# nii-yamagishilab/NELE-GAN

Measured on AMD Instinct MI355X. Metric: utterances/sec per GAN_epoch step (G+D+metric loss), higher is better.
Workload: dtype bf16

## Files before the change

nele_gan_amd/_lib.py:

```python
import ctypes
import os

import torch

from . import _abi, _abi_ext, _abi_ext2, _abi_ext3

FUNCS = dict(_abi.FUNCS, **_abi_ext.FUNCS)
CONSTS = dict(_abi.CONSTS, **_abi_ext.CONSTS)
FUNCS2 = dict(_abi_ext2.FUNCS)
CONSTS2 = dict(_abi_ext2.CONSTS)
FUNCS3 = dict(_abi_ext3.FUNCS)
CONSTS3 = dict(_abi_ext3.CONSTS)

_HERE = os.path.dirname(os.path.abspath(__file__))
LIB_PATH = os.environ.get('NELE_LIB') or os.path.join(_HERE, 'libnele_hip.so')

c_int = ctypes.c_int
c_float = ctypes.c_float
c_double = ctypes.c_double
c_void_p = ctypes.c_void_p
c_size_t = ctypes.c_size_t
c_longlong = ctypes.c_longlong


class NeleError(RuntimeError):
    pass


def _load():
    if not os.path.exists(LIB_PATH):
        raise ImportError(
            "nele_gan_amd: %s not found -- build it with `python -c 'import __graft_entry__ as g; g.build()'` "
            "or `make -C nele_gan_amd/csrc` (hipcc, gfx950). There is no fallback path." % LIB_PATH)
    return ctypes.CDLL(LIB_PATH)


lib = _load()


def _bind(every):
    missing = sorted(n for n in every if not hasattr(lib, n))
    if missing:
        raise ImportError("nele_gan_amd: %s does not export %s (declared in include/nele_hip*.h) -- "
                          "rebuild it with `python -c 'import __graft_entry__ as g; g.build()'`" % (LIB_PATH, ', '.join(missing)))
    sigs = {}
    for name, (restype, argtypes) in every.items():
        fn = getattr(lib, name)
        fn.restype = getattr(ctypes, 'c_' + restype)
        fn.argtypes = sigs[name] = [getattr(ctypes, 'c_' + a) for a in argtypes]
    return sigs


_SIGS = _bind(dict(FUNCS, **FUNCS2))
_SIGS3 = _bind(FUNCS3)


def check(status, name=''):
    if status != 0:
        msg = lib.nele_last_error_string().decode('utf-8', 'replace')
        if status == -1:
            raise ValueError("%s: %s" % (name, msg))
        raise NeleError("%s failed (status %d): %s" % (name, status, msg))


PLAN_MAXARGS = CONSTS['NELE_PLAN_MAXARGS']


class nele_plan_job(ctypes.Structure):
    _fields_ = [('op', c_int), ('nargs', c_int), ('stream', c_int), ('slot', c_int * PLAN_MAXARGS), ('ival', c_longlong * PLAN_MAXARGS),
                ('fval', c_double * PLAN_MAXARGS)]


def call(name, *args):
    check(getattr(lib, name)(*args), name)


def ptr(t):
    if t is None:
        return None
    if not t.is_cuda:
        raise ValueError("nele_gan_amd: expected a tensor on the GPU (got %s)" % t.device)
    if not t.is_contiguous():
        raise ValueError("nele_gan_amd: expected a contiguous tensor")
    return c_void_p(t.data_ptr())


def norm_dev(dev):
    dev = torch.device(dev)
    if dev.type == 'cuda' and dev.index is None:
        dev = torch.device('cuda', torch.cuda.current_device())
    return dev


_raw_stream = getattr(torch._C, '_cuda_getCurrentRawStream', None)
_raw_device = getattr(torch._C, '_cuda_getDevice', None)


def stream():
    if _raw_stream is not None and _raw_device is not None:
        return c_void_p(_raw_stream(_raw_device()))
    return c_void_p(torch.cuda.current_stream().cuda_stream)


def profile_begin(tag):
    lib.nele_profile_begin(tag.encode() if tag else None)


# ... 19 lines not shown
```

nele_gan_amd/csrc/conv16.hip:

```cpp
#include "conv_common.h"
#include <cstdlib>
#include <cstring>
#include <type_traits>

#define C16_TW 64
#ifndef C16_SB
#define C16_SB 4
#endif

#ifdef C16_PROF
__device__ unsigned long long c16_prof[8];
#define C16_T(var) const unsigned long long var = __builtin_readcyclecounter()
#define C16_ACC(slot, t0_, t1_) do { c16_acc[slot] += (t1_) - (t0_); } while (0)
#else
#define C16_T(var) do {} while (0)
#define C16_ACC(slot, t0_, t1_) do {} while (0)
#endif

struct Conv16Args {
    const __bf16* A;
    const __bf16* Wfrag;
    const float* bias;
    const __bf16* aux;
    void* out;
    int N, epi;
    float slope;
    int KH, KW, sps, nsteps;
    int RSP, NR;
    int lgC, swz_sh, swz_mask;
    int ntiles, TH;
    double* gap;
    const int* wvalid;
    ConvGeom g;
};

__device__ __forceinline__ void c16_dma(const __bf16* gsrc_lane, __bf16* lds_piece) {
    __builtin_amdgcn_global_load_lds((const __attribute__((address_space(1))) void*)gsrc_lane, (__attribute__((address_space(3))) void*)lds_piece, 16, 0, 0);
}

template <int TN, int TH, bool OUT16>
__global__ __launch_bounds__(256, 2) void conv16_kernel(Conv16Args p) {
    C16_T(t_start);
#ifdef C16_PROF
    unsigned long long c16_acc[5] = {0, 0, 0, 0, 0};
#endif
    extern __shared__ __attribute__((aligned(16))) __bf16 lds16[];
    const ConvGeom& g = p.g;
    const int tid = threadIdx.x, lane = tid & 63, li = lane & 15, lg = lane >> 4;
    const int wave = __builtin_amdgcn_readfirstlane(tid >> 6);
    int wo0, ho0, b;
    {
        const int ntw = (g.Wout + C16_TW - 1) / C16_TW, nth = (g.Hout + TH - 1) / TH;
        const int per = (int)((gridDim.x + 7) >> 3);
        const int tile = (int)(blockIdx.x & 7) * per + (int)(blockIdx.x >> 3);
        if (tile >= p.ntiles) return;
        const int tw_i = tile % ntw, rem = tile / ntw;
        wo0 = tw_i * C16_TW; ho0 = (rem % nth) * TH; b = rem / nth;
    }
    const int C = g.C, RSP = p.RSP, NR = p.NR;
    const int wcols = C16_TW + p.KW - 1;
    const int nrows = TH + p.KH - 1;
    const int hi0 = ho0 + g.ih0, wi0 = wo0 + g.iw0;
    const int vcols = max(1, min(wcols, g.W - wi0));
    const int vrows = max(1, min(nrows, g.H - hi0));
    const __bf16* abase = p.A + (((size_t)b * g.H + hi0) * g.W + wi0) * C;
    __bf16* wring = lds16 + NR * RSP + 64;
    constexpr int CH = C16_SB * TN * 512;

    const int npieces = RSP >> 9;
    int rsrc[3];
#pragma unroll
    for (int t = 0; t < 3; ++t) {
        const int o = 512 * (wave + 4 * t) + 8 * lane;
        const int q = o / C, un = ((o - q * C) >> 3) ^ ((q >> p.swz_sh) & p.swz_mask);
        rsrc[t] = min(q, vcols - 1) * C + 8 * un;
    }
    auto row_dma = [&](int r) {
        const __bf16* src = abase + (size_t)min(r, vrows - 1) * g.W * C;
        __bf16* dst = lds16 + (r % NR) * RSP;
#pragma unroll
        for (int t = 0; t < 3; ++t)
            if (wave + 4 * t < npieces) c16_dma(src + rsrc[t], dst + 512 * (wave + 4 * t));
    };
    const int nchunk = (p.nsteps + C16_SB - 1) / C16_SB;
    const __bf16* wsrc = p.Wfrag + 512 * wave + 8 * lane;
    auto w_dma = [&](int c) {
        const __bf16* src = wsrc + (size_t)c * CH;
        __bf16* dst = wring + (c & 1) * CH + 512 * wave;
#pragma unroll
        for (int q = 0; q < (C16_SB * TN + 3) / 4; ++q)
            if ((C16_SB * TN) % 4 == 0 || wave + 4 * q < C16_SB * TN) c16_dma(src + 2048 * q, dst + 2048 * q);
    };
    int resident = min(NR, nrows) - 1;
    for (int r = 0; r <= resident; ++r) row_dma(r);
    w_dma(0);
    if (tid < 8) *reinterpret_cast<bf16x8*>(lds16 + NR * RSP + 8 * tid) = (bf16x8){(__bf16)0.f, (__bf16)0.f, (__bf16)0.f, (__bf16)0.f, (__bf16)0.f, (__bf16)0.f, (__bf16)0.f, (__bf16)0.f};

    const int nr = min(TH, g.Hout - ho0), ncol = min(4, (g.Wout - wo0 + 15) >> 4), total = nr * ncol;
    const int NPr = (total + 3) >> 2;
    const int n0 = 4 * TN * lg;
    const int vb = li * C;

    auto run = [&](auto np_tag) {
        constexpr int NP = decltype(np_tag)::value;
        int prow[NP], pcol[NP];
        bool pok[NP];
#pragma unroll
        for (int k = 0; k < NP; ++k) {
            int t = wave + 4 * k;
            pok[k] = t < total;
            if (!pok[k]) t -= total;
            if (t >= total) t %= total;
            prow[k] = t / ncol; pcol[k] = t - prow[k] * ncol;
        }
        f32x4 acc[NP][TN];
#pragma unroll
        for (int k = 0; k < NP; ++k)
#pragma unroll
            for (int j = 0; j < TN; ++j) acc[k][j] = (f32x4){0.f, 0.f, 0.f, 0.f};
        __builtin_amdgcn_s_waitcnt(0x0f70);
        __syncthreads();
        C16_T(t_pro);
        C16_ACC(1, t_start, t_pro);

        int lu = 0, rr[NP], so[NP];
#pragma unroll
        for (int k = 0; k < NP; ++k) { rr[k] = prow[k]; so[k] = prow[k] * RSP + 16 * pcol[k] * C; }
        const __bf16* wl = wring + lane * 8;
        auto ldfrag = [&](int uu, bf16x8 (&af)[NP], bf16x8 (&bfr)[TN]) {
            const int kk8 = lu * 32 + 8 * lg;
            const int vk = (vb + kk8) ^ ((((li + (kk8 >> p.lgC)) >> p.swz_sh) & p.swz_mask) << 3);
#pragma unroll
            for (int j = 0; j < TN; ++j) bfr[j] = *reinterpret_cast<const bf16x8*>(wl + (uu * TN + j) * 512);
#pragma unroll
            for (int k = 0; k < NP; ++k) af[k] = *reinterpret_cast<const bf16x8*>(lds16 + so[k] + vk);
            if (__builtin_expect(++lu == p.sps, 0)) {
                asm volatile("" ::: "memory");
                lu = 0;
#pragma unroll
                for (int k = 0; k < NP; ++k) {
                    so[k] += RSP;
                    if (++rr[k] == NR) { rr[k] = 0; so[k] -= NR * RSP; }
                }
            }
        };
        auto mm = [&](const bf16x8 (&af)[NP], const bf16x8 (&bfr)[TN]) {
#pragma unroll
            for (int k = 0; k < NP; ++k)
#pragma unroll
                for (int j = 0; j < TN; ++j) acc[k][j] = __builtin_amdgcn_mfma_f32_16x16x32_bf16(bfr[j], af[k], acc[k][j], 0, 0, 0);
        };
        constexpr int MPR = (NP * TN) / (NP + TN) > 0 ? (NP * TN) / (NP + TN) : 1;
#define C16_INTERLEAVE()                                                                  \
    _Pragma("unroll") for (int q_ = 0; q_ < NP + TN; ++q_) {                              \
        __builtin_amdgcn_sched_group_barrier(0x008, MPR, 0);                              \
        __builtin_amdgcn_sched_group_barrier(0x100, 1, 0);                                \
        __builtin_amdgcn_sched_group_barrier(0x002, 3, 0);                                \
    }                                                                                     \
    __builtin_amdgcn_sched_group_barrier(0x008, NP * TN, 0);                              \
    __builtin_amdgcn_sched_barrier(0);                                                    \
    __builtin_amdgcn_s_waitcnt(0xc07f);                                                   \
    __builtin_amdgcn_sched_barrier(0)
        const int nfull = p.nsteps / C16_SB, nrem = p.nsteps - nfull * C16_SB;
        int nl_row = (2 * C16_SB - 1) / p.sps, nl_rem = (2 * C16_SB - 1) - nl_row * p.sps;
        for (int c = 0; c < nfull; ++c) {
            if (c + 1 < nchunk) {
                w_dma(c + 1);
                const int need = min(nl_row + TH - 1, nrows - 1);
                if (need > resident) { ++resident; row_dma(resident); }
                nl_rem += C16_SB;
                while (nl_rem >= p.sps) { nl_rem -= p.sps; ++nl_row; }
            }
            bf16x8 a0[NP], b0[TN], a1[NP], b1[TN];
            ldfrag(0, a0, b0);
            __builtin_amdgcn_sched_barrier(0);
            __builtin_amdgcn_s_waitcnt(0xc07f);
            __builtin_amdgcn_sched_barrier(0);
#pragma unroll
            for (int uu = 0; uu + 1 < C16_SB; ++uu) {
                if (uu & 1) { ldfrag(uu + 1, a0, b0); mm(a1, b1); }
                else { ldfrag(uu + 1, a1, b1); mm(a0, b0); }
                C16_INTERLEAVE();
            }
            if (C16_SB & 1) mm(a0, b0); else mm(a1, b1);
            wl += (c & 1) ? -CH : CH;
            if (c + 1 < nchunk) {
                C16_T(t_w0);
                __builtin_amdgcn_s_waitcnt(0x0f70);
                C16_T(t_w1);
                __syncthreads();
                C16_T(t_w2);
                C16_ACC(2, t_w0, t_w1);
                C16_ACC(3, t_w1, t_w2);
            }
        }
#undef C16_INTERLEAVE
        for (int uu = 0; uu < nrem; ++uu) {
            bf16x8 a0[NP], b0[TN];
            ldfrag(uu, a0, b0);
            mm(a0, b0);
        }

        C16_T(t_epi);
        float bv[4 * TN];
#pragma unroll
        for (int q = 0; q < 4 * TN; ++q)
            bv[q] = ((p.epi == EPI_BIAS || p.epi == EPI_BIAS_LRELU) && n0 + q < p.N) ? p.bias[n0 + q] : 0.f;
        const bool pool = p.gap != nullptr;
        const int wpool = pool ? (p.wvalid ? min(p.wvalid[b], g.Wout) : g.Wout) : 0;
        double gs[4 * TN];
#pragma unroll
        for (int q = 0; q < 4 * TN; ++q) gs[q] = 0.0;
#pragma unroll
        for (int k = 0; k < NP; ++k) {
            const int ho = ho0 + prow[k], wo = wo0 + 16 * pcol[k] + li;
            if (!pok[k] || wo >= g.Wout || n0 >= p.N) continue;
            float v[4 * TN];
#pragma unroll
            for (int j = 0; j < TN; ++j)
#pragma unroll
                for (int reg = 0; reg < 4; ++reg) v[4 * j + reg] = acc[k][j][reg] + bv[4 * j + reg];
            if (p.epi == EPI_BIAS_LRELU) {
#pragma unroll
                for (int q = 0; q < 4 * TN; ++q) v[q] = v[q] > 0.f ? v[q] : p.slope * v[q];
                if (pool && wo < wpool) {
#pragma unroll
                    for (int q = 0; q < 4 * TN; ++q) gs[q] += (double)v[q];
                }
            } else if (p.epi == EPI_MASK_LRELU_GRAD) {
                const __bf16* xp = p.aux + (((size_t)b * g.Hout + ho) * g.Wout + wo) * p.N + n0;
#pragma unroll
                for (int j = 0; j < TN; ++j) {
                    if (n0 + 4 * j < p.N) {
                        const bf16x4 x = *reinterpret_cast<const bf16x4*>(xp + 4 * j);
#pragma unroll
                        for (int reg = 0; reg < 4; ++reg) v[4 * j + reg] = (float)x[reg] > 0.f ? v[4 * j + reg] : p.slope * v[4 * j + reg];
                    }
                }
            }
            const size_t o_off = (((size_t)b * g.OH + ho + g.oh0) * g.OW + wo + g.ow0) * g.OC + n0;
            if (OUT16) {
                __bf16* op = reinterpret_cast<__bf16*>(p.out) + o_off;
#pragma unroll
                for (int j = 0; j < TN; ++j) {
                    if (n0 + 4 * j < p.N) {
                        bf16x4 h;
#pragma unroll
                        for (int reg = 0; reg < 4; ++reg) h[reg] = (__bf16)v[4 * j + reg];
                        *reinterpret_cast<bf16x4*>(op + 4 * j) = h;
                    }
                }
            } else {
                float* op = reinterpret_cast<float*>(p.out) + o_off;
#pragma unroll
                for (int j = 0; j < TN; ++j)
                    if (n0 + 4 * j < p.N) *reinterpret_cast<float4*>(op + 4 * j) = make_float4(v[4 * j], v[4 * j + 1], v[4 * j + 2], v[4 * j + 3]);
            }
        }
        if (pool) {
            const int ntw_ = (g.Wout + C16_TW - 1) / C16_TW, nth_ = (g.Hout + TH - 1) / TH;
            const int part = ((ho0 / TH) * ntw_ + wo0 / C16_TW) * 4 + wave;
            double* gp = p.gap + ((size_t)b * (ntw_ * nth_ * 4) + part) * p.N + n0;
#pragma unroll
            for (int q = 0; q < 4 * TN; ++q) {
                const double t = row16_sum_dpp(gs[q]);
                if (li == 0 && n0 + q < p.N) gp[q] = t;
            }
        }
        C16_T(t_end);
        C16_ACC(4, t_epi, t_end);
        C16_ACC(0, t_start, t_end);
#ifdef C16_PROF
        if (threadIdx.x == 0) { for (int q_ = 0; q_ < 5; ++q_) atomicAdd(&c16_prof[q_], c16_acc[q_]); atomicAdd(&c16_prof[5], 1ull); }
#endif
    };
    if (TH == 8) {
        switch (NPr) {
            case 8: run(std::integral_constant<int, (TH == 8 ? 8 : 1)>{}); break;
            case 7: run(std::integral_constant<int, (TH == 8 ? 7 : 1)>{}); break;
            case 6: run(std::integral_constant<int, (TH == 8 ? 6 : 1)>{}); break;
            case 5: run(std::integral_constant<int, (TH == 8 ? 5 : 1)>{}); break;
            case 4: run(std::integral_constant<int, 4>{}); break;
            case 3: run(std::integral_constant<int, 3>{}); break;
            case 2: run(std::integral_constant<int, 2>{}); break;
            default: run(std::integral_constant<int, 1>{}); break;
        }
    } else {
        switch (NPr) {
            case 4: run(std::integral_constant<int, 4>{}); break;
            case 3: run(std::integral_constant<int, 3>{}); break;
            case 2: run(std::integral_constant<int, 2>{}); break;
            default: run(std::integral_constant<int, 1>{}); break;
        }
    }
}

__global__ __launch_bounds__(256) void conv16_pointwise_kernel(const float4* __restrict__ in, const float* __restrict__ W, const float* __restrict__ bias,
                                                               __bf16* __restrict__ out, long long M, float slope) {
    __shared__ float w[8][4], bs[8];
    if (threadIdx.x < 32) w[threadIdx.x >> 2][threadIdx.x & 3] = W[threadIdx.x];
    if (threadIdx.x < 8) bs[threadIdx.x] = bias[threadIdx.x];
    __syncthreads();
    for (long long m = (long long)blockIdx.x * 256 + threadIdx.x; m < M; m += (long long)gridDim.x * 256) {
        const float4 a = in[m];
        bf16x8 h;
#pragma unroll
        for (int n = 0; n < 8; ++n) {
            float v = fmaf(a.w, w[n][3], fmaf(a.y, w[n][1], fmaf(a.z, w[n][2], a.x * w[n][0]))) + bs[n];
            v = v > 0.f ? v : slope * v;
            h[n] = (__bf16)v;
        }
        *reinterpret_cast<bf16x8*>(out + 8 * m) = h;
    }
}

extern "C" int nele_conv16_pointwise_fwd(const float* in, const float* Wf, const float* bias, void* out16, long long M, int N, float slope, void* stream) {
    NELE_CHECK_ARG(in && Wf && bias && out16 && M > 0 && N == 8, "nele_conv16_pointwise_fwd: needs 4 -> 8 channels");
    const long long blocks = (M + 255) / 256;
    hipLaunchKernelGGL(conv16_pointwise_kernel, dim3((unsigned)(blocks < 8192 ? blocks : 8192)), dim3(256), 0, as_stream(stream),
                       reinterpret_cast<const float4*>(in), Wf, bias, reinterpret_cast<__bf16*>(out16), M, slope);
    NELE_CHECK_LAUNCH("conv16_pointwise_kernel");
    return NELE_OK;
}

struct C16FragJobs { const float* Wg[16]; __bf16* Wfrag[16]; int N[16], Ktot[16], seglen[16], KH[16]; };
__global__ void conv16_frag_kernel(C16FragJobs J) {
    const int job = blockIdx.y;
    const float* __restrict__ Wg = J.Wg[job];
    __bf16* __restrict__ Wf = J.Wfrag[job];
    const int N = J.N[job], Ktot = J.Ktot[job], seglen = J.seglen[job], KH = J.KH[job];
    const int TN = (N + 15) >> 4, sps = (seglen + 31) >> 5;
    const long long total = (long long)(KH * sps + C16_SB) * TN * 512;
    for (long long idx = (long long)blockIdx.x * blockDim.x + threadIdx.x; idx < total; idx += (long long)gridDim.x * blockDim.x) {
        const int e = (int)(idx & 7), lane = (int)((idx >> 3) & 63);
        const long long f = idx >> 9;
        const int j = (int)(f % TN), s = (int)(f / TN);
        const int m = lane & 15, gq = lane >> 4;
        const int n = 4 * TN * (m >> 2) + 4 * j + (m & 3);
        float v = 0.f;
        if (s < KH * sps && n < N) {
            const int kh = s / sps, us = s - kh * sps;
            const int ko = us * 32 + 8 * gq + e;
            if (ko < seglen) v = Wg[(size_t)n * Ktot + kh * seglen + ko];
        }
        Wf[idx] = (__bf16)v;
    }
}

struct C16Plan { int TN, TH, NR, RSP, lgC, swz_sh, swz_mask, sps; size_t lds; };
static bool c16_plan(int N, const ConvGeom& g, int KH, int KW, C16Plan* pl, int epi = EPI_NONE) {
    if (N < 4 || N > 64 || (N & 3) || g.C < 8 || g.C > 64 || (g.C & 7) || KH < 2 || KW < 2 || KW > 9 || KH > 9) return false;
    if (g.seglen != KW * g.C || g.Ktot != KH * KW * g.C) return false;
    C16Plan q;
    q.TN = (N + 15) >> 4;
    q.sps = (g.seglen + 31) >> 5;
    const int nsteps = KH * q.sps;
    int th = (nsteps * q.TN <= 64 && q.TN <= 2) ? 8 : 4;
    if (epi == EPI_MASK_LRELU_GRAD) th = 4;
    q.TH = th;
    q.lgC = 0; q.swz_sh = 0; q.swz_mask = 0;
    if (g.C == 64) { q.lgC = 6; q.swz_mask = 7; }
    else if (g.C == 32) { q.lgC = 5; q.swz_sh = 1; q.swz_mask = 3; }
    q.RSP = ((C16_TW + KW - 1) * g.C + 511) & ~511;
    if (q.RSP > 12 * 512) return false;
    const int full = q.TH + KH - 1;
    const int ring = q.sps >= 2 * C16_SB - 1 ? q.TH + 1 : q.sps >= C16_SB ? q.TH + 2 : full;
    q.NR = ring < full ? ring : full;
    q.lds = ((size_t)q.NR * q.RSP + 64 + 2 * C16_SB * q.TN * 512) * 2;
    if (q.lds > 160 * 1024) return false;
    *pl = q;
    return true;
}

#ifdef C16_PROF
extern "C" int nele_conv16_prof_read(unsigned long long* out8, int reset) {
    if (hipDeviceSynchronize() != hipSuccess) return 1;
    if (hipMemcpyFromSymbol(out8, HIP_SYMBOL(c16_prof), sizeof(unsigned long long) * 8) != hipSuccess) return 1;
    if (reset) { unsigned long long z[8] = {0}; if (hipMemcpyToSymbol(HIP_SYMBOL(c16_prof), z, sizeof(z)) != hipSuccess) return 1; }
    return 0;
}
#endif

extern "C" int nele_conv16_supported(int M, int N, const int* geom, int KH, int KW) {
    ConvGeom g;
    memcpy(&g, geom, sizeof(ConvGeom));
    C16Plan pl;
    return c16_plan(N, g, KH, KW, &pl) ? 1 : 0;
}

extern "C" long long nele_conv16_wfrag_elems(int N, int seglen, int KH) {
    const int TN = (N + 15) >> 4, sps = (seglen + 31) >> 5;
    return (long long)(KH * sps + C16_SB) * TN * 512;
}

extern "C" int nele_conv16_weight_prep_batch(const void* const* ptrs_host, const int* dims_host, int jobs, void* stream) {
    NELE_CHECK_ARG(ptrs_host && dims_host && jobs >= 1 && jobs <= 16, "nele_conv16_weight_prep_batch: 1..16 jobs");
    C16FragJobs J;
    long long mx = 0;
    for (int i = 0; i < jobs; ++i) {
        J.Wg[i] = (const float*)ptrs_host[2 * i]; J.Wfrag[i] = (__bf16*)ptrs_host[2 * i + 1];
        J.N[i] = dims_host[4 * i]; J.Ktot[i] = dims_host[4 * i + 1]; J.seglen[i] = dims_host[4 * i + 2]; J.KH[i] = dims_host[4 * i + 3];
        NELE_CHECK_ARG(J.Wg[i] && J.Wfrag[i] && J.Ktot[i] == J.seglen[i] * J.KH[i], "nele_conv16_weight_prep_batch: bad job %d", i);
        const long long t = nele_conv16_wfrag_elems(J.N[i], J.seglen[i], J.KH[i]);
        if (t > mx) mx = t;
    }
    const int blocks = (int)((mx + 255) / 256 < 512 ? (mx + 255) / 256 : 512);
    hipLaunchKernelGGL(conv16_frag_kernel, dim3(blocks, jobs), dim3(256), 0, as_stream(stream), J);
    NELE_CHECK_LAUNCH("conv16_frag_kernel");
    return NELE_OK;
}

template <int TN, int TH, bool OUT16>
static void c16_launch(const Conv16Args& a, dim3 grid, size_t lds, hipStream_t s) {
    static unsigned long long attr = 0;
    if (nele_first_use_on_device(&attr)) {
        (void)hipFuncSetAttribute(reinterpret_cast<const void*>(conv16_kernel<TN, TH, OUT16>), hipFuncAttributeMaxDynamicSharedMemorySize, 160 * 1024);
    }
    hipLaunchKernelGGL((conv16_kernel<TN, TH, OUT16>), grid, dim3(256), lds, s, a);
}

static int conv16_impl(const void* A16, const void* Wfrag, const float* bias, const void* aux16, void* out, int out_bf16, int M, int N, int epi,
                       float slope, const int* geom, int KH, int KW, const int* wvalid, double* gap_part, void* stream) {
    NELE_CHECK_ARG(A16 && Wfrag && out && geom, "nele_conv16: null pointer");
    ConvGeom g;
    memcpy(&g, geom, sizeof(ConvGeom));
    C16Plan pl;
    if (!c16_plan(N, g, KH, KW, &pl, epi)) return nele_set_error(NELE_ERR_UNSUPPORTED, "nele_conv16: unsupported geometry (C %d N %d %dx%d)", g.C, N, KH, KW);
    NELE_CHECK_ARG(epi == EPI_NONE || epi == EPI_BIAS || epi == EPI_BIAS_LRELU || epi == EPI_MASK_LRELU_GRAD, "nele_conv16: epilogue %d", epi);
    NELE_CHECK_ARG(epi != EPI_MASK_LRELU_GRAD || aux16, "nele_conv16: the mask epilogue needs the forward activation");
    NELE_CHECK_ARG((epi != EPI_BIAS && epi != EPI_BIAS_LRELU) || bias, "nele_conv16: bias missing");
    NELE_CHECK_ARG(g.Hout > 0 && g.Wout > 0 && M % (g.Hout * g.Wout) == 0, "nele_conv16: M is not a multiple of Hout * Wout");
    NELE_CHECK_ARG((g.OC & 3) == 0, "nele_conv16: output channel stride must be a multiple of 4");
    const int B = M / (g.Hout * g.Wout);
    Conv16Args a;
    a.A = (const __bf16*)A16; a.Wfrag = (const __bf16*)Wfrag; a.bias = bias; a.aux = (const __bf16*)aux16; a.out = out;
    a.N = N; a.epi = epi; a.slope = slope; a.KH = KH; a.KW = KW; a.sps = pl.sps; a.nsteps = KH * pl.sps;
    a.RSP = pl.RSP; a.NR = pl.NR; a.lgC = pl.lgC; a.swz_sh = pl.swz_sh; a.swz_mask = pl.swz_mask; a.TH = pl.TH; a.g = g;
    a.gap = gap_part; a.wvalid = wvalid;
    a.ntiles = ((g.Wout + C16_TW - 1) / C16_TW) * ((g.Hout + pl.TH - 1) / pl.TH) * B;
    const dim3 grid((unsigned)((a.ntiles + 7) / 8 * 8));
    hipStream_t s = as_stream(stream);
#define C16_GO(TN_, TH_) do { if (out_bf16) c16_launch<TN_, TH_, true>(a, grid, pl.lds, s); else c16_launch<TN_, TH_, false>(a, grid, pl.lds, s); } while (0)
#define C16_PICK(TH_) switch (pl.TN) { case 1: C16_GO(1, TH_); break; case 2: C16_GO(2, TH_); break; case 3: C16_GO(3, TH_); break; default: C16_GO(4, TH_); break; }
    char ptag[48] = "conv16_kernel";
    if (nele_prof_armed() && !nele_prof_match("conv16_kernel")) snprintf(ptag, sizeof(ptag), "conv16_N%d_K%d_e%d", N, g.Ktot, epi);
    NELE_PROF(ptag, s, if (pl.TH == 8) { C16_PICK(8); } else { C16_PICK(4); });
#undef C16_PICK
#undef C16_GO
    NELE_CHECK_LAUNCH("conv16_kernel");
    return NELE_OK;
}

extern "C" int nele_conv16(const void* A16, const void* Wfrag, const float* bias, const void* aux16, void* out, int out_bf16, int M, int N, int epi,
                           float slope, const int* geom, int KH, int KW, void* stream) {
    return conv16_impl(A16, Wfrag, bias, aux16, out, out_bf16, M, N, epi, slope, geom, KH, KW, nullptr, nullptr, stream);
}

extern "C" int nele_conv16_gap_parts(int N, const int* geom, int KH, int KW) {
    if (!geom) return 0;
    ConvGeom g;
    memcpy(&g, geom, sizeof(ConvGeom));
    C16Plan pl;
    if (!c16_plan(N, g, KH, KW, &pl, EPI_BIAS_LRELU)) return 0;
    return ((g.Wout + C16_TW - 1) / C16_TW) * ((g.Hout + pl.TH - 1) / pl.TH) * 4;
}

extern "C" int nele_conv16_gap(const void* A16, const void* Wfrag, const float* bias, void* out16, int M, int N, float slope, const int* geom, int KH,
                               int KW, const int* wvalid, double* gap_part, void* stream) {
    NELE_CHECK_ARG(gap_part, "nele_conv16_gap: null pointer");
    return conv16_impl(A16, Wfrag, bias, nullptr, out16, 1, M, N, EPI_BIAS_LRELU, slope, geom, KH, KW, wvalid, gap_part, stream);
}
```

nele_gan_amd/csrc/netplan.hip:

```cpp
#include "common.h"
#include "conv_common.h"
#include "ws_arena.h"
#include "../../include/nele_hip.h"
#include <cstring>
#include <initializer_list>
#include <memory>
#include <vector>

int nele_plan_adopt(void* plan, std::vector<std::unique_ptr<char[]>>&& blobs, std::vector<hipEvent_t>&& events);

namespace {

constexpr double SLOPE = 0.3;

struct Geom { int a[15]; int KH, KW, Hout, Wout, Ktot; };
Geom mk_geom(int H, int W, int C, int Hout, int Wout, int KH, int KW, int OH, int OW, int OC, int ih0 = 0, int iw0 = 0, int oh0 = 0, int ow0 = 0) {
    Geom g;
    const int v[15] = {H, W, C, ih0, iw0, Hout, Wout, KW * C, W * C, KH * KW * C, OH, OW, OC, oh0, ow0};
    memcpy(g.a, v, sizeof(v));
    g.KH = KH; g.KW = KW; g.Hout = Hout; g.Wout = Wout; g.Ktot = KH * KW * C;
    return g;
}

struct Buf { void* p = nullptr; long long elems = 0; bool b16 = false; };
// ... 518 lines not shown

void d_backward(Builder& b, const DWs& w, const float* par, float* grad, const DParams& pp, const void* const* uv, int B, int T, int cin, int nout, bool bf16,
                bool need_din, bool wgrad, bool overlap) {
    const void* const* mlp = d_mlp_ptrs(b, w, par, pp);
    const int Ho = w.dims[5][0], Wo = w.dims[5][1], p5 = w.pad[4];
    const bool g16 = bf16 && (w.grad16_ok || w.c16);
    const Buf& glast = (g16 && !w.c16) ? w.gbuf16 : w.gbuf[4];
    b.add(g16 ? (w.c16 ? "nele_gap_mlp_bwd_var16a" : "nele_gap_mlp_bwd_var16") : "nele_gap_mlp_bwd_var", 0,
          {S(0), S(1), P(w.h1), P(w.h2), P(w.act[4]), P(mlp), I(nout), F(SLOPE), I(B), I(Ho), I(Wo), S(2), I(Ho + 2 * p5), I(Wo + 2 * p5), I(p5), I(p5), P(w.dz3), P(w.dz2),
           P(w.dz1), P(w.dpooled), P(glast)});
    if (overlap) { b.hand_over(0, 1); b.hand_over(0, 2); }
    const float* sig = reinterpret_cast<const float*>(w.sigma.p);
    if (wgrad) {
        const int st = overlap ? 2 : 0;
        const Buf& tw = overlap ? w.tmpw2 : w.tmpw;
        const Buf& sc = overlap ? w.scratch64b : w.scratch64;
        const Buf* dz[3] = {&w.dz3, &w.dz2, &w.dz1};
        const Buf* xin[3] = {&w.h2, &w.h1, &w.pooled};
        for (int i = 0; i < 3; ++i) {
            const int li = 7 - i, N = pp.N[li], K = pp.K[li];
            float* tmpb = reinterpret_cast<float*>(tw.p) + (long long)N * K;
            b.add("nele_mlp_wgrad", st, {P(*dz[i]), P(*xin[i]), I(B), I(N), I(K), P(tw), P(tmpb)});
            b.add("nele_sn_grad", st, {P(tw), P(par + pp.w[li]), P(uv[2 * li]), P(uv[2 * li + 1]), P(sig + li), I(N), I(K), P(grad + pp.w[li]), I(1), P(sc)});
            b.add("nele_vec_add", st, {P(grad + pp.bias[li]), P(tmpb), I(N)});
        }
    }
    Buf din; din.elems = (long long)B * 64 * T * 4;
    for (int l = 4; l >= 0; --l) {
        const int co = D_CONVS[l][0], k = D_CONVS[l][1];
        const int Ci = w.dims[l][2];
        const int cin_valid = l == 0 ? cin : Ci;
        if (wgrad) {
            const int N = co, K = cin_valid * k * k;
            const int q = l == 0 ? 1 : (l & 1);
            const Buf& tw = q == 0 ? w.tmpw : w.tmpw2;
            const Buf& wsb = q == 0 ? w.ws : w.ws2;
            const Buf& sc = q == 0 ? w.scratch64 : w.scratch64b;
            float* tmpb = reinterpret_cast<float*>(tw.p) + (long long)N * K;
            const int st = overlap ? 1 + q : 0;
            if (overlap) b.hand_over(0, st);
            const Buf& dOut = l == 4 ? glast : w.gbuf[l];
            const bool b16 = bf16 && l > 0;
            const char* fn = b16 ? "nele_conv_wgrad_bf16" : (w.x3 && l > 0) ? "nele_conv_wgrad_bf16x3" : "nele_conv_wgrad";
            const bool a16 = l > 0 && w.act[l - 1].b16;
            if (dOut.b16) fn = a16 ? "nele_conv_wgrad_bf16_a16d16" : "nele_conv_wgrad_bf16_d16";
            const Geom& g = w.gw[l];
            b.add(fn, st, {l == 0 ? S(3) : P(w.act[l - 1]), P(dOut), P(wsb), I(wsb.elems), I(M_of(B, g)), I(co), P(b.geom(g)), I(g.KH), I(g.KW), I(cin_valid), P(tw), P(tmpb), I(0)});
            b.add("nele_sn_grad", st, {P(tw), P(par + pp.w[l]), P(uv[2 * l]), P(uv[2 * l + 1]), P(sig + l), I(N), I(K), P(grad + pp.w[l]), I(1), P(sc)});
            b.add("nele_vec_add", st, {P(grad + pp.bias[l]), P(tmpb), I(N)});
        }
        const Geom& g = w.gb[l];
        const long long M = M_of(B, g);
        if (l > 0 && w.c16) {
            b.add("nele_conv16", 0, {P(w.gbuf[l]), P(w.wb16c[l]), P((void*)nullptr), P(w.act[l - 1]), P(w.gbuf[l - 1]), I(w.gbuf[l - 1].b16 ? 1 : 0), I(M), I(Ci), I(EPI_MASK_LRELU_GRAD),
                                    F(SLOPE), P(b.geom(g)), I(g.KH), I(g.KW)});
        } else if (l > 0) {
            if (w.x3_b[l]) {
                b.add("nele_conv_span_bf16x3", 0, {P(w.gbuf[l]), P(w.wbx3[l][0]), P(w.wbx3[l][1]), P((void*)nullptr), P(w.act[l - 1]), P(w.gbuf[l - 1]), I(M), I(Ci),
                                                    I(EPI_MASK_LRELU_GRAD), F(SLOPE), P(b.geom(g)), I(g.KH), I(g.KW), I(w.gbuf[l].elems)});
            } else if (bf16 && w.span16_b[l]) {
                const Buf& src = l == 4 ? glast : w.gbuf[l];
                b.add(src.b16 ? "nele_conv_span_bf16_a16" : "nele_conv_span_bf16", 0, {P(src), P(w.wbf16[l]), P((void*)nullptr), P(w.act[l - 1]), P(w.gbuf[l - 1]), I(M), I(Ci),
                                                                                    I(EPI_MASK_LRELU_GRAD), F(SLOPE), P(b.geom(g)), I(g.KH), I(g.KW), I(src.elems)});
            } else if (w.span_b[l]) {
                b.add("nele_conv_span", 0, {P(w.gbuf[l]), P(w.wbf[l]), P((void*)nullptr), P(w.act[l - 1]), P(w.gbuf[l - 1]), I(M), I(Ci), I(EPI_MASK_LRELU_GRAD), F(SLOPE), P(b.geom(g)),
                                           I(g.KH), I(g.KW), I(w.gbuf[l].elems)});
            } else {
                b.add("nele_conv_gemm", 0, {P(w.gbuf[l]), P(w.wb[l]), P((void*)nullptr), P(w.act[l - 1]), P(w.gbuf[l - 1]), I(M), I(Ci), I(EPI_MASK_LRELU_GRAD), F(SLOPE), P(b.geom(g))});
            }
        } else if (need_din) {
            b.add("nele_conv_gemm", 0, {P(w.gbuf[0]), P(w.wb[0]), P((void*)nullptr), P((void*)nullptr), P(w.ddin), I(M), I(4), I(EPI_NONE), F(SLOPE), P(b.geom(g))});
        }
    }
    if (overlap) { b.hand_over(1, 0); b.hand_over(2, 0); }
}

}

static bool prec_bf16(int prec) { return prec != NELE_PREC_F32 && prec != NELE_PREC_BF16X3; }
static bool prec_x3(int prec) { return prec == NELE_PREC_BF16X3; }

extern "C" long long nele_gen_param_count(void) { return g_params().total; }
extern "C" long long nele_disc_param_count(int cin, int nout) { return (cin >= 1 && cin <= 4 && nout >= 1 && nout <= 4) ? d_params(cin, nout).total : -1; }

extern "C" int nele_gen_param_layout(long long* offsets, int n) {
    NELE_CHECK_ARG(offsets && n >= 28, "nele_gen_param_layout: 28 offsets");
    const GParams p = g_params();
    int k = 0;
    for (int l = 0; l < 6; ++l) { offsets[k++] = p.w[l]; offsets[k++] = p.b[l]; offsets[k++] = p.gain[l]; offsets[k++] = p.beta[l]; }
    for (int q = 0; q < 2; ++q) { offsets[k++] = p.fcw[q]; offsets[k++] = p.fcb[q]; }
    return k;
}
extern "C" int nele_disc_param_layout(int cin, int nout, long long* offsets, int n) {
    NELE_CHECK_ARG(offsets && n >= 16 && cin >= 1 && cin <= 4 && nout >= 1 && nout <= 4, "nele_disc_param_layout: 16 offsets, cin 1..4, nout 1..4");
    const DParams p = d_params(cin, nout);
    int k = 0;
    for (int l = 0; l < 8; ++l) { offsets[k++] = p.bias[l]; offsets[k++] = p.w[l]; }
    return k;
}

extern "C" long long nele_gen_workspace_bytes(int B, int T, int bf16, int need_bwd) {
    if (B <= 0 || T <= 0) return -1;
    GWs w;
    g_layout(B, T, prec_bf16(bf16), need_bwd != 0, nullptr, w, prec_x3(bf16));
    return (long long)w.bytes;
}

namespace {
// ... 149 lines not shown
```

nele_gan_amd/csrc/plan.hip:

```cpp
#include "common.h"
#include "../../include/nele_hip.h"
#include <cstring>
#include <memory>
#include <new>
#include <vector>

struct PlanJobI {
    int op, nargs, stream;
    int slot[NELE_PLAN_MAXARGS];
    long long ival[NELE_PLAN_MAXARGS];
    double fval[NELE_PLAN_MAXARGS];
};
struct NelePlan {
    unsigned magic;
    int nslots, nstreams;
    std::vector<PlanJobI> jobs;
    long long slot_bytes[64];
    unsigned char slot_nullable[64];
    std::vector<std::unique_ptr<char[]>> blobs;
    std::vector<hipEvent_t> events;
    ~NelePlan() { for (hipEvent_t e : events) (void)hipEventDestroy(e); }
};
#define PLAN_MAGIC 0x4e504c4eu

struct PlanOpInfo { const char* name; int nargs; };
static const PlanOpInfo plan_ops[] = {
#define PLAN_OP_TABLE
#define PLAN_OP(idx, name, nargs) {#name, nargs},
#include "plan_ops.inc"
#undef PLAN_OP
#undef PLAN_OP_TABLE
};
static const int plan_nops = (int)(sizeof(plan_ops) / sizeof(plan_ops[0]));

extern "C" int nele_plan_op_id(const char* name) {
    if (!name) return -1;
    for (int k = 0; k < plan_nops; ++k)
        if (!strcmp(plan_ops[k].name, name)) return k;
    return -1;
}
extern "C" int nele_plan_op_nargs(int op) { return (op >= 0 && op < plan_nops) ? plan_ops[op].nargs : -1; }

static int plan_dispatch(int op, const long long* v, const double* d, void* S) {
#define V(i) v[i]
#define D(i) d[i]
    switch (op) {
#define PLAN_OP_CASES
#include "plan_ops.inc"
#undef PLAN_OP_CASES
        default: break;
    }
#undef V
#undef D
    return nele_set_error(NELE_ERR_INVALID_ARG, "nele_plan_run: unknown operation %d", op);
}

extern "C" int nele_plan_create(const nele_plan_job* jobs, int njobs, int nslots, int nstreams, void** plan_out) {
    NELE_CHECK_ARG(jobs && njobs > 0 && nslots >= 0 && nslots <= 64 && nstreams >= 1 && nstreams <= 16 && plan_out, "nele_plan_create: bad arguments");
    for (int j = 0; j < njobs; ++j) {
        const nele_plan_job& q = jobs[j];
        NELE_CHECK_ARG(q.op >= 0 && q.op < plan_nops, "nele_plan_create: job %d: unknown operation %d", j, q.op);
        NELE_CHECK_ARG(q.nargs == plan_ops[q.op].nargs, "nele_plan_create: job %d (%s): %d arguments, the entry point takes %d", j, plan_ops[q.op].name, q.nargs,
                       plan_ops[q.op].nargs);
        NELE_CHECK_ARG(q.stream >= 0 && q.stream < nstreams, "nele_plan_create: job %d: stream %d of %d", j, q.stream, nstreams);
        for (int i = 0; i + 1 < q.nargs; ++i)
            NELE_CHECK_ARG(q.slot[i] >= -1 && q.slot[i] < nslots, "nele_plan_create: job %d argument %d: slot %d of %d", j, i, q.slot[i], nslots);
    }
    NelePlan* p = new (std::nothrow) NelePlan;
    if (!p) return nele_set_error(NELE_ERR_HIP, "nele_plan_create: out of host memory");
    p->magic = PLAN_MAGIC; p->nslots = nslots; p->nstreams = nstreams;
    memset(p->slot_bytes, 0, sizeof(p->slot_bytes)); memset(p->slot_nullable, 0, sizeof(p->slot_nullable));
    p->jobs.resize(njobs);
    for (int j = 0; j < njobs; ++j) {
        PlanJobI& o = p->jobs[j];
        o.op = jobs[j].op; o.nargs = jobs[j].nargs; o.stream = jobs[j].stream;
        memcpy(o.slot, jobs[j].slot, sizeof(o.slot)); memcpy(o.ival, jobs[j].ival, sizeof(o.ival)); memcpy(o.fval, jobs[j].fval, sizeof(o.fval));
    }
    *plan_out = p;
    return NELE_OK;
}

extern "C" int nele_plan_declare_slot(void* plan, int slot, long long bytes, int nullable) {
    NelePlan* p = reinterpret_cast<NelePlan*>(plan);
    NELE_CHECK_ARG(p && p->magic == PLAN_MAGIC && slot >= 0 && slot < p->nslots && bytes >= 0, "nele_plan_declare_slot: bad arguments");
    p->slot_bytes[slot] = bytes; p->slot_nullable[slot] = nullable ? 1 : 0;
    return NELE_OK;
}
extern "C" long long nele_plan_slot_bytes(void* plan, int slot) {
    NelePlan* p = reinterpret_cast<NelePlan*>(plan);
    if (!p || p->magic != PLAN_MAGIC || slot < 0 || slot >= p->nslots) return -1;
    return p->slot_bytes[slot];
}

int nele_plan_adopt(void* plan, std::vector<std::unique_ptr<char[]>>&& blobs, std::vector<hipEvent_t>&& events) {
    NelePlan* p = reinterpret_cast<NelePlan*>(plan);
    if (!p || p->magic != PLAN_MAGIC) return nele_set_error(NELE_ERR_INVALID_ARG, "nele_plan_adopt: not a plan");
    p->blobs = std::move(blobs); p->events = std::move(events);
    return NELE_OK;
}

extern "C" int nele_plan_destroy(void* plan) {
    NelePlan* p = reinterpret_cast<NelePlan*>(plan);
    if (!p || p->magic != PLAN_MAGIC) return nele_set_error(NELE_ERR_INVALID_ARG, "nele_plan_destroy: not a plan");
    p->magic = 0;
// ... 81 lines not shown
```

Measured before the change: 7437.

## Skip zero-padded border rows in conv16 backward-data kernel

Adds a zero-border variant of the conv16 kernel, used for the masked LReLU gradient convolution in the network plan. Each tile narrows its kernel-row range to the rows that touch real (non-padded) input, cuts the step count and offsets the weight fragments to match, so MACs and DMA against zero padding rows are skipped. It also packs per-piece row and column metadata into one 64-bit word for the TH=8 path, simplifies the ring-index wrap, and compiles only even piece counts for that path to trim registers and template instances. The zero-border path forces TH=4, which may reduce reuse for some layers.

```diff
diff --git a/include/nele_hip_ext4.h b/include/nele_hip_ext4.h
--- /dev/null
+++ b/include/nele_hip_ext4.h
@@ -0,0 +1,13 @@
+#ifndef NELE_HIP_EXT4_H
+#define NELE_HIP_EXT4_H
+#ifdef __cplusplus
+extern "C" {
+#endif
+
+int nele_conv16_zb(const void* A16, const void* Wfrag, const float* bias, const void* aux16, void* out, int out_bf16, int M, int N, int epi,
+                   float slope, const int* geom_host, int KH, int KW, int zrows, void* stream);
+
+#ifdef __cplusplus
+}
+#endif
+#endif
diff --git a/nele_gan_amd/_abi_ext4.py b/nele_gan_amd/_abi_ext4.py
--- /dev/null
+++ b/nele_gan_amd/_abi_ext4.py
@@ -0,0 +1,5 @@
+CONSTS = {
+}
+FUNCS = {
+    'nele_conv16_zb': ('int', ('void_p', 'void_p', 'void_p', 'void_p', 'void_p', 'int', 'int', 'int', 'int', 'float', 'void_p', 'int', 'int', 'int', 'void_p')),
+}
diff --git a/nele_gan_amd/_lib.py b/nele_gan_amd/_lib.py
--- a/nele_gan_amd/_lib.py
+++ b/nele_gan_amd/_lib.py
@@ -3,7 +3,7 @@
 
 import torch
 
-from . import _abi, _abi_ext, _abi_ext2, _abi_ext3
+from . import _abi, _abi_ext, _abi_ext2, _abi_ext3, _abi_ext4
 
 FUNCS = dict(_abi.FUNCS, **_abi_ext.FUNCS)
 CONSTS = dict(_abi.CONSTS, **_abi_ext.CONSTS)
@@ -11,6 +11,8 @@
 CONSTS2 = dict(_abi_ext2.CONSTS)
 FUNCS3 = dict(_abi_ext3.FUNCS)
 CONSTS3 = dict(_abi_ext3.CONSTS)
+FUNCS4 = dict(_abi_ext4.FUNCS)
+CONSTS4 = dict(_abi_ext4.CONSTS)
 
 _HERE = os.path.dirname(os.path.abspath(__file__))
 LIB_PATH = os.environ.get('NELE_LIB') or os.path.join(_HERE, 'libnele_hip.so')
@@ -53,6 +55,7 @@
 
 _SIGS = _bind(dict(FUNCS, **FUNCS2))
 _SIGS3 = _bind(FUNCS3)
+_SIGS4 = _bind(FUNCS4)
 
 
 def check(status, name=''):
diff --git a/nele_gan_amd/csrc/conv16.hip b/nele_gan_amd/csrc/conv16.hip
--- a/nele_gan_amd/csrc/conv16.hip
+++ b/nele_gan_amd/csrc/conv16.hip
@@ -1,4 +1,5 @@
 #include "conv_common.h"
+#include "../../include/nele_hip_ext4.h"
 #include <cstdlib>
 #include <cstring>
 #include <type_traits>
@@ -32,14 +33,17 @@
     double* gap;
     const int* wvalid;
     ConvGeom g;
+    int zrows;
 };
 
 __device__ __forceinline__ void c16_dma(const __bf16* gsrc_lane, __bf16* lds_piece) {
     __builtin_amdgcn_global_load_lds((const __attribute__((address_space(1))) void*)gsrc_lane, (__attribute__((address_space(3))) void*)lds_piece, 16, 0, 0);
 }
 
-template <int TN, int TH, bool OUT16>
+template <int TN, int THZ, bool OUT16>
 __global__ __launch_bounds__(256, 2) void conv16_kernel(Conv16Args p) {
+    constexpr bool ZB = THZ < 0;
+    constexpr int TH = ZB ? -THZ : THZ;
     C16_T(t_start);
 #ifdef C16_PROF
     unsigned long long c16_acc[5] = {0, 0, 0, 0, 0};
@@ -59,8 +63,18 @@
     }
     const int C = g.C, RSP = p.RSP, NR = p.NR;
     const int wcols = C16_TW + p.KW - 1;
-    const int nrows = TH + p.KH - 1;
-    const int hi0 = ho0 + g.ih0, wi0 = wo0 + g.iw0;
+    int hi0 = ho0 + g.ih0, nkh = 0, wskip = 0;
+    if (ZB) {
+        const int nr = min(TH, g.Hout - ho0);
+        const int kh_lo = min(p.KH - 1, max(0, p.zrows - (hi0 + nr - 1)));
+        const int kh_hi = min(p.KH - 1, g.H - p.zrows - 1 - hi0);
+        nkh = max(0, kh_hi - kh_lo + 1);
+        hi0 += kh_lo;
+        wskip = kh_lo * p.sps;
+    }
+    const int nsteps = ZB ? nkh * p.sps : p.nsteps;
+    const int nrows = TH + (ZB ? max(nkh, 1) : p.KH) - 1;
+    const int wi0 = wo0 + g.iw0;
     const int vcols = max(1, min(wcols, g.W - wi0));
     const int vrows = max(1, min(nrows, g.H - hi0));
     const __bf16* abase = p.A + (((size_t)b * g.H + hi0) * g.W + wi0) * C;
@@ -82,8 +96,8 @@
         for (int t = 0; t < 3; ++t)
             if (wave + 4 * t < npieces) c16_dma(src + rsrc[t], dst + 512 * (wave + 4 * t));
     };
-    const int nchunk = (p.nsteps + C16_SB - 1) / C16_SB;
-    const __bf16* wsrc = p.Wfrag + 512 * wave + 8 * lane;
+    const int nchunk = (nsteps + C16_SB - 1) / C16_SB;
+    const __bf16* wsrc = p.Wfrag + (ZB ? (size_t)wskip * (TN * 512) : (size_t)0) + 512 * wave + 8 * lane;
     auto w_dma = [&](int c) {
         const __bf16* src = wsrc + (size_t)c * CH;
         __bf16* dst = wring + (c & 1) * CH + 512 * wave;
@@ -113,6 +127,12 @@
             if (t >= total) t %= total;
             prow[k] = t / ncol; pcol[k] = t - prow[k] * ncol;
         }
+        constexpr bool LEAN = TH == 8;
+        unsigned long long ppack = 0;
+        if (LEAN) {
+#pragma unroll
+            for (int k = 0; k < NP; ++k) ppack |= (unsigned long long)(prow[k] | (pcol[k] << 3) | ((int)pok[k] << 5)) << (6 * k);
+        }
         f32x4 acc[NP][TN];
 #pragma unroll
         for (int k = 0; k < NP; ++k)
@@ -140,7 +160,8 @@
 #pragma unroll
                 for (int k = 0; k < NP; ++k) {
                     so[k] += RSP;
-                    if (++rr[k] == NR) { rr[k] = 0; so[k] -= NR * RSP; }
+                    if (LEAN) { if (so[k] >= NR * RSP) so[k] -= NR * RSP; }
+                    else if (++rr[k] == NR) { rr[k] = 0; so[k] -= NR * RSP; }
                 }
             }
         };
@@ -161,7 +182,7 @@
     __builtin_amdgcn_sched_barrier(0);                                                    \
     __builtin_amdgcn_s_waitcnt(0xc07f);                                                   \
     __builtin_amdgcn_sched_barrier(0)
-        const int nfull = p.nsteps / C16_SB, nrem = p.nsteps - nfull * C16_SB;
+        const int nfull = nsteps / C16_SB, nrem = nsteps - nfull * C16_SB;
         int nl_row = (2 * C16_SB - 1) / p.sps, nl_rem = (2 * C16_SB - 1) - nl_row * p.sps;
         for (int c = 0; c < nfull; ++c) {
             if (c + 1 < nchunk) {
@@ -213,8 +234,11 @@
         for (int q = 0; q < 4 * TN; ++q) gs[q] = 0.0;
 #pragma unroll
         for (int k = 0; k < NP; ++k) {
-            const int ho = ho0 + prow[k], wo = wo0 + 16 * pcol[k] + li;
-            if (!pok[k] || wo >= g.Wout || n0 >= p.N) continue;
+            const unsigned pf = (unsigned)(ppack >> (6 * k));
+            const int prow_k = LEAN ? (int)(pf & 7) : prow[k], pcol_k = LEAN ? (int)((pf >> 3) & 3) : pcol[k];
+            const bool pok_k = LEAN ? ((pf >> 5) & 1) != 0 : pok[k];
+            const int ho = ho0 + prow_k, wo = wo0 + 16 * pcol_k + li;
+            if (!pok_k || wo >= g.Wout || n0 >= p.N) continue;
             float v[4 * TN];
 #pragma unroll
             for (int j = 0; j < TN; ++j)
@@ -275,15 +299,11 @@
 #endif
     };
     if (TH == 8) {
-        switch (NPr) {
-            case 8: run(std::integral_constant<int, (TH == 8 ? 8 : 1)>{}); break;
-            case 7: run(std::integral_constant<int, (TH == 8 ? 7 : 1)>{}); break;
-            case 6: run(std::integral_constant<int, (TH == 8 ? 6 : 1)>{}); break;
-            case 5: run(std::integral_constant<int, (TH == 8 ? 5 : 1)>{}); break;
-            case 4: run(std::integral_constant<int, 4>{}); break;
-            case 3: run(std::integral_constant<int, 3>{}); break;
-            case 2: run(std::integral_constant<int, 2>{}); break;
-            default: run(std::integral_constant<int, 1>{}); break;
+        switch ((NPr + 1) >> 1) {
+            case 4: run(std::integral_constant<int, (TH == 8 ? 8 : 1)>{}); break;
+            case 3: run(std::integral_constant<int, (TH == 8 ? 6 : 1)>{}); break;
+            case 2: run(std::integral_constant<int, 4>{}); break;
+            default: run(std::integral_constant<int, 2>{}); break;
         }
     } else {
         switch (NPr) {
@@ -348,7 +368,7 @@
 }
 
 struct C16Plan { int TN, TH, NR, RSP, lgC, swz_sh, swz_mask, sps; size_t lds; };
-static bool c16_plan(int N, const ConvGeom& g, int KH, int KW, C16Plan* pl, int epi = EPI_NONE) {
+static bool c16_plan(int N, const ConvGeom& g, int KH, int KW, C16Plan* pl, int epi = EPI_NONE, int zrows = 0) {
     if (N < 4 || N > 64 || (N & 3) || g.C < 8 || g.C > 64 || (g.C & 7) || KH < 2 || KW < 2 || KW > 9 || KH > 9) return false;
     if (g.seglen != KW * g.C || g.Ktot != KH * KW * g.C) return false;
     C16Plan q;
@@ -356,7 +376,7 @@
     q.sps = (g.seglen + 31) >> 5;
     const int nsteps = KH * q.sps;
     int th = (nsteps * q.TN <= 64 && q.TN <= 2) ? 8 : 4;
-    if (epi == EPI_MASK_LRELU_GRAD) th = 4;
+    if (epi == EPI_MASK_LRELU_GRAD || zrows > 0) th = 4;
     q.TH = th;
     q.lgC = 0; q.swz_sh = 0; q.swz_mask = 0;
     if (g.C == 64) { q.lgC = 6; q.swz_mask = 7; }
@@ -420,12 +440,13 @@
 }
 
 static int conv16_impl(const void* A16, const void* Wfrag, const float* bias, const void* aux16, void* out, int out_bf16, int M, int N, int epi,
-                       float slope, const int* geom, int KH, int KW, const int* wvalid, double* gap_part, void* stream) {
+                       float slope, const int* geom, int KH, int KW, const int* wvalid, double* gap_part, int zrows, void* stream) {
     NELE_CHECK_ARG(A16 && Wfrag && out && geom, "nele_conv16: null pointer");
     ConvGeom g;
     memcpy(&g, geom, sizeof(ConvGeom));
     C16Plan pl;
-    if (!c16_plan(N, g, KH, KW, &pl, epi)) return nele_set_error(NELE_ERR_UNSUPPORTED, "nele_conv16: unsupported geometry (C %d N %d %dx%d)", g.C, N, KH, KW);
+    NELE_CHECK_ARG(zrows >= 0 && zrows < KH && 2 * zrows <= g.H, "nele_conv16_zb: zrows %d is not a border of a %d-row image under a %d-row kernel", zrows, g.H, KH);
+    if (!c16_plan(N, g, KH, KW, &pl, epi, zrows)) return nele_set_error(NELE_ERR_UNSUPPORTED, "nele_conv16: unsupported geometry (C %d N %d %dx%d)", g.C, N, KH, KW);
     NELE_CHECK_ARG(epi == EPI_NONE || epi == EPI_BIAS || epi == EPI_BIAS_LRELU || epi == EPI_MASK_LRELU_GRAD, "nele_conv16: epilogue %d", epi);
     NELE_CHECK_ARG(epi != EPI_MASK_LRELU_GRAD || aux16, "nele_conv16: the mask epilogue needs the forward activation");
     NELE_CHECK_ARG((epi != EPI_BIAS && epi != EPI_BIAS_LRELU) || bias, "nele_conv16: bias missing");
@@ -436,16 +457,22 @@
     a.A = (const __bf16*)A16; a.Wfrag = (const __bf16*)Wfrag; a.bias = bias; a.aux = (const __bf16*)aux16; a.out = out;
     a.N = N; a.epi = epi; a.slope = slope; a.KH = KH; a.KW = KW; a.sps = pl.sps; a.nsteps = KH * pl.sps;
     a.RSP = pl.RSP; a.NR = pl.NR; a.lgC = pl.lgC; a.swz_sh = pl.swz_sh; a.swz_mask = pl.swz_mask; a.TH = pl.TH; a.g = g;
-    a.gap = gap_part; a.wvalid = wvalid;
+    a.gap = gap_part; a.wvalid = wvalid; a.zrows = zrows;
     a.ntiles = ((g.Wout + C16_TW - 1) / C16_TW) * ((g.Hout + pl.TH - 1) / pl.TH) * B;
     const dim3 grid((unsigned)((a.ntiles + 7) / 8 * 8));
+    bool zb = false;
+    for (int ho0 = 0; zrows > 0 && ho0 < g.Hout && !zb; ho0 += pl.TH) {
+        const int hi0 = ho0 + g.ih0, nr = g.Hout - ho0 < pl.TH ? g.Hout - ho0 : pl.TH;
+        zb = zrows - (hi0 + nr - 1) > 0 || g.H - zrows - 1 - hi0 < KH - 1;
+    }
     hipStream_t s = as_stream(stream);
 #define C16_GO(TN_, TH_) do { if (out_bf16) c16_launch<TN_, TH_, true>(a, grid, pl.lds, s); else c16_launch<TN_, TH_, false>(a, grid, pl.lds, s); } while (0)
-#define C16_PICK(TH_) switch (pl.TN) { case 1: C16_GO(1, TH_); break; case 2: C16_GO(2, TH_); break; case 3: C16_GO(3, TH_); break; default: C16_GO(4, TH_); break; }
     char ptag[48] = "conv16_kernel";
     if (nele_prof_armed() && !nele_prof_match("conv16_kernel")) snprintf(ptag, sizeof(ptag), "conv16_N%d_K%d_e%d", N, g.Ktot, epi);
-    NELE_PROF(ptag, s, if (pl.TH == 8) { C16_PICK(8); } else { C16_PICK(4); });
-#undef C16_PICK
+    NELE_PROF(ptag, s,
+              if (zb) { switch (pl.TN) { case 1: C16_GO(1, -4); break; case 2: C16_GO(2, -4); break; case 3: C16_GO(3, -4); break; default: C16_GO(4, -4); break; } }
+              else if (pl.TH == 8) { if (pl.TN == 1) C16_GO(1, 8); else C16_GO(2, 8); }
+              else { switch (pl.TN) { case 1: C16_GO(1, 4); break; case 2: C16_GO(2, 4); break; case 3: C16_GO(3, 4); break; default: C16_GO(4, 4); break; } });
 #undef C16_GO
     NELE_CHECK_LAUNCH("conv16_kernel");
     return NELE_OK;
@@ -453,7 +480,12 @@
 
 extern "C" int nele_conv16(const void* A16, const void* Wfrag, const float* bias, const void* aux16, void* out, int out_bf16, int M, int N, int epi,
                            float slope, const int* geom, int KH, int KW, void* stream) {
-    return conv16_impl(A16, Wfrag, bias, aux16, out, out_bf16, M, N, epi, slope, geom, KH, KW, nullptr, nullptr, stream);
+    return conv16_impl(A16, Wfrag, bias, aux16, out, out_bf16, M, N, epi, slope, geom, KH, KW, nullptr, nullptr, 0, stream);
+}
+
+extern "C" int nele_conv16_zb(const void* A16, const void* Wfrag, const float* bias, const void* aux16, void* out, int out_bf16, int M, int N, int epi,
+                              float slope, const int* geom, int KH, int KW, int zrows, void* stream) {
+    return conv16_impl(A16, Wfrag, bias, aux16, out, out_bf16, M, N, epi, slope, geom, KH, KW, nullptr, nullptr, zrows, stream);
 }
 
 extern "C" int nele_conv16_gap_parts(int N, const int* geom, int KH, int KW) {
@@ -468,5 +500,5 @@
 extern "C" int nele_conv16_gap(const void* A16, const void* Wfrag, const float* bias, void* out16, int M, int N, float slope, const int* geom, int KH,
                                int KW, const int* wvalid, double* gap_part, void* stream) {
     NELE_CHECK_ARG(gap_part, "nele_conv16_gap: null pointer");
-    return conv16_impl(A16, Wfrag, bias, nullptr, out16, 1, M, N, EPI_BIAS_LRELU, slope, geom, KH, KW, wvalid, gap_part, stream);
-}
+    return conv16_impl(A16, Wfrag, bias, nullptr, out16, 1, M, N, EPI_BIAS_LRELU, slope, geom, KH, KW, wvalid, gap_part, 0, stream);
+}
diff --git a/nele_gan_amd/csrc/netplan.hip b/nele_gan_amd/csrc/netplan.hip
--- a/nele_gan_amd/csrc/netplan.hip
+++ b/nele_gan_amd/csrc/netplan.hip
@@ -594,8 +594,8 @@
         const Geom& g = w.gb[l];
         const long long M = M_of(B, g);
         if (l > 0 && w.c16) {
-            b.add("nele_conv16", 0, {P(w.gbuf[l]), P(w.wb16c[l]), P((void*)nullptr), P(w.act[l - 1]), P(w.gbuf[l - 1]), I(w.gbuf[l - 1].b16 ? 1 : 0), I(M), I(Ci), I(EPI_MASK_LRELU_GRAD),
-                                    F(SLOPE), P(b.geom(g)), I(g.KH), I(g.KW)});
+            b.add("nele_conv16_zb", 0, {P(w.gbuf[l]), P(w.wb16c[l]), P((void*)nullptr), P(w.act[l - 1]), P(w.gbuf[l - 1]), I(w.gbuf[l - 1].b16 ? 1 : 0), I(M), I(Ci),
+                                       I(EPI_MASK_LRELU_GRAD), F(SLOPE), P(b.geom(g)), I(g.KH), I(g.KW), I(w.pad[l])});
         } else if (l > 0) {
             if (w.x3_b[l]) {
                 b.add("nele_conv_span_bf16x3", 0, {P(w.gbuf[l]), P(w.wbx3[l][0]), P(w.wbx3[l][1]), P((void*)nullptr), P(w.act[l - 1]), P(w.gbuf[l - 1]), I(M), I(Ci),
diff --git a/nele_gan_amd/csrc/plan.hip b/nele_gan_amd/csrc/plan.hip
--- a/nele_gan_amd/csrc/plan.hip
+++ b/nele_gan_amd/csrc/plan.hip
@@ -1,5 +1,6 @@
 #include "common.h"
 #include "../../include/nele_hip.h"
+#include "../../include/nele_hip_ext4.h"
 #include <cstring>
 #include <memory>
 #include <new>
@@ -30,8 +31,10 @@
 #include "plan_ops.inc"
 #undef PLAN_OP
 #undef PLAN_OP_TABLE
+    {"nele_conv16_zb", 15},
 };
 static const int plan_nops = (int)(sizeof(plan_ops) / sizeof(plan_ops[0]));
+#define PLAN_OP_CONV16_ZB (plan_nops - 1)
 
 extern "C" int nele_plan_op_id(const char* name) {
     if (!name) return -1;
@@ -50,6 +53,10 @@
 #undef PLAN_OP_CASES
         default: break;
     }
+    if (op == PLAN_OP_CONV16_ZB)
+        return nele_conv16_zb((const void*)(uintptr_t)V(0), (const void*)(uintptr_t)V(1), (const float*)(uintptr_t)V(2), (const void*)(uintptr_t)V(3),
+                              (void*)(uintptr_t)V(4), (int)V(5), (int)V(6), (int)V(7), (int)V(8), (float)D(9), (const int*)(uintptr_t)V(10), (int)V(11),
+                              (int)V(12), (int)V(13), S);
 #undef V
 #undef D
     return nele_set_error(NELE_ERR_INVALID_ARG, "nele_plan_run: unknown operation %d", op);
```

Result: no change. 7428, median of 3 (-0.1%).
